# mpt0816/Cilqr

Hardware: AMD Instinct MI355X
Metric: CILQR solves/sec (50-step horizon, batch=65536 per GPU) (higher is better)
Workload: dtype f64

## Files before the change

cilqr_amd/csrc/backward_core.hpp:

```cpp
#pragma once
#include "dev_model.hpp"

namespace cilqr {

__host__ __device__ constexpr int a_kind(int r, int c) {
  return (r == c) ? 1
         : ((r == 0 || r == 1) && c >= 2) ? 2
         : (r == 2 && c >= 3) ? 2
         : (r == 3 && c == 4) ? 2
         : 0;
}
__host__ __device__ constexpr int b_kind(int r, int c) {
  return ((r == 2 && c == 1) || (r == 3 && c == 0) || (r == 4 && c == 0) || (r == 5 && c == 1)) ? 2 : 0;
}
__host__ __device__ constexpr int h_kind(int r, int c) {
  return (r < 3 && c < 3) ? 2 : (r == c) ? 2 : 0;
}

#define ACC_TERM(acc, t)            \
  do {                              \
    if ((acc).any) (acc).v += (t);  \
    else { (acc).v = (t); (acc).any = true; } \
  } while (0)

// ... 14 lines not shown
      const Acc a = acc_sum6_xty(t);
      out[r * xcols + c] = a.any ? a.v : 0.0;
    }
}
template <int C, int rows, bool IsA>
CILQR_DEV void x_m(const double* __restrict__ X, const double* __restrict__ M, double* out) {
#pragma unroll
  for (int r = 0; r < rows; ++r)
#pragma unroll
    for (int c = 0; c < C; ++c) {
      Acc a{0.0, false};
#pragma unroll
      for (int k = 0; k < 6; ++k) {
        const int kind = IsA ? a_kind(k, c) : b_kind(k, c);
        if (kind == 0) continue;
        const double x = X[r * 6 + k];
        const double t = (kind == 1) ? x : x * M[k * C + c];
        ACC_TERM(a, t);
      }
      out[r * C + c] = a.any ? a.v : 0.0;
    }
}

template <bool kStore>
CILQR_DEV void backward_problem(const DeviceState& s, int slot, double lambda, double2* stage) {
  const Params& p = s.p;
  const int Bc = s.Bcap, N = p.N;
  const double dt = p.dt;
  const int sp = scratch_index(s, slot);
  double Vx[6], Vxx[36];
  {
    const double2* t = s.term + sp;
    const double2 t0 = t[0], t1 = t[(size_t)Bc], t2 = t[(size_t)2 * Bc], t3 = t[(size_t)3 * Bc],
                  t4 = t[(size_t)4 * Bc], t5 = t[(size_t)5 * Bc], t6 = t[(size_t)6 * Bc],
                  t7 = t[(size_t)7 * Bc], t8 = t[(size_t)8 * Bc];
    Vx[0] = t0.x; Vx[1] = t0.y; Vx[2] = t1.x; Vx[3] = t1.y; Vx[4] = t2.x; Vx[5] = t2.y;
#pragma unroll
    for (int e = 0; e < 36; ++e) Vxx[e] = 0.0;
    Vxx[0] = t3.x; Vxx[1] = t3.y; Vxx[2] = t4.x;
    Vxx[6] = t4.y; Vxx[7] = t5.x; Vxx[8] = t5.y;
    Vxx[12] = t6.x; Vxx[13] = t6.y; Vxx[14] = t7.x;
    Vxx[21] = t7.y; Vxx[28] = t8.x; Vxx[35] = t8.y;
  }
  const int buf = s.cur[slot];
  double dV0 = 0.0, dV1 = 0.0, gsum = 0.0;
  double2 w[kLinPairs];
  double2 uu;
  constexpr int kRows = kLinPairs + 1;
  auto fetch_to_lds = [&](int step) {
    using gptr = const __attribute__((address_space(1))) void*;
    using lptr = __attribute__((address_space(3))) void*;
    const double2* q = s.lin + (size_t)step * kLinPairs * Bc + sp;
    double2* dst = stage + (size_t)(step & 1) * kRows * 64;
#pragma unroll
    for (int r = 0; r < kLinPairs; ++r)
      __builtin_amdgcn_global_load_lds((gptr)(q + (size_t)r * Bc), (lptr)(dst + r * 64), 16, 0, 0);
    __builtin_amdgcn_global_load_lds((gptr)(s.U + ((size_t)buf * N + step) * Bc + slot), (lptr)(dst + kLinPairs * 64), 16, 0, 0);
  };
  fetch_to_lds(N - 1);
  for (int i = N - 1; i >= 0; --i) {
    {
      asm volatile("s_waitcnt vmcnt(0)" ::: "memory");
      const double2* src = stage + (size_t)(i & 1) * kRows * 64 + (threadIdx.x & 63);
#pragma unroll
      for (int r = 0; r < kLinPairs; ++r) w[r] = src[r * 64];
      uu = src[kLinPairs * 64];
      if (i > 0) fetch_to_lds(i - 1);
    }
    double A[36], B[12];
    A[2] = w[0].x; A[3] = w[0].y; A[4] = w[1].x; A[5] = w[1].y;
    A[8] = w[2].x; A[9] = w[2].y; A[10] = w[3].x; A[11] = w[3].y;
    A[15] = w[4].x; A[16] = w[4].y; A[17] = w[5].x;
    A[22] = dt;
    B[5] = w[5].y; B[6] = 0.5 * dt * dt; B[8] = dt; B[11] = dt;
    const double lx[6] = {w[6].x, w[6].y, w[7].x, w[7].y, w[8].x, w[8].y};
    const double lu[2] = {w[9].x, w[9].y};
    double H[36];
    H[0] = w[10].x; H[1] = w[10].y; H[2] = w[11].x;
    H[6] = w[11].y; H[7] = w[12].x; H[8] = w[12].y;
    H[12] = w[13].x; H[13] = w[13].y; H[14] = w[14].x;
    H[21] = w[14].y; H[28] = w[15].x; H[35] = w[15].y;
    const double luu0 = w[16].x, luu1 = w[16].y;

    double BtV[12], Qux[12], BtVB[4], BtVx[2];
    mt_x<2, 6, false>(B, Vxx, BtV);
    x_m<6, 2, true>(BtV, A, Qux);
    x_m<2, 2, false>(BtV, B, BtVB);
    mt_x<2, 1, false>(B, Vx, BtVx);
    const double Quu[4] = {luu0 + BtVB[0], BtVB[1], BtVB[2], luu1 + BtVB[3]};
    const double Qu[2] = {lu[0] + BtVx[0], lu[1] + BtVx[1]};
    const double m00 = Quu[0] + lambda, m01 = Quu[1], m10 = Quu[2], m11 = Quu[3] + lambda;
    const double invdet = 1.0 / (m00 * m11 - m10 * m01);
    const double n00 = -(m11 * invdet), n01 = -(-m01 * invdet), n10 = -(-m10 * invdet),
                 n11 = -(m00 * invdet);
    double Kc[12], kc[2];
#pragma unroll
    for (int c = 0; c < 6; ++c) {
      Kc[c] = n00 * Qux[c] + n01 * Qux[6 + c];
      Kc[6 + c] = n10 * Qux[c] + n11 * Qux[6 + c];
    }
    kc[0] = n00 * Qu[0] + n01 * Qu[1];
    kc[1] = n10 * Qu[0] + n11 * Qu[1];
    if (kStore) {
      double2* g = s.gains + (size_t)i * kGainPairs * Bc + sp;
#pragma unroll
      for (int r = 0; r < 6; ++r) g[(size_t)r * Bc] = make_double2(Kc[2 * r], Kc[2 * r + 1]);
      g[(size_t)6 * Bc] = make_double2(kc[0], kc[1]);
    }
    {
      const double v0 = fabs(kc[0]) / (fabs(uu.x) + 1), v1 = fabs(kc[1]) / (fabs(uu.y) + 1);
      gsum += (v0 > v1 ? v0 : v1);
    }
    double AtVx[6], AtV[36], AtVA[36];
    mt_x<6, 1, true>(A, Vx, AtVx);
    mt_x<6, 6, true>(A, Vxx, AtV);
    x_m<6, 6, true>(AtV, A, AtVA);
    double KtQ[12];
#pragma unroll
    for (int r = 0; r < 6; ++r) {
      KtQ[r * 2 + 0] = Kc[r] * Quu[0] + Kc[6 + r] * Quu[2];
      KtQ[r * 2 + 1] = Kc[r] * Quu[1] + Kc[6 + r] * Quu[3];
    }
    double nVx[6];
#pragma unroll
    for (int r = 0; r < 6; ++r) {
      const double t1 = KtQ[r * 2] * kc[0] + KtQ[r * 2 + 1] * kc[1];
      const double t2 = Kc[r] * Qu[0] + Kc[6 + r] * Qu[1];
      const double t3 = Qux[r] * kc[0] + Qux[6 + r] * kc[1];
      nVx[r] = (((lx[r] + AtVx[r]) + t1) + t2) + t3;
    }
#pragma unroll
    for (int r = 0; r < 6; ++r)
#pragma unroll
      for (int c = 0; c < 6; ++c) {
        const double m1 = KtQ[r * 2] * Kc[c] + KtQ[r * 2 + 1] * Kc[6 + c];
        const double m2 = Kc[r] * Qux[c] + Kc[6 + r] * Qux[6 + c];
        const double m3 = Qux[r] * Kc[c] + Qux[6 + r] * Kc[6 + c];
        const double qxx = (h_kind(r, c) == 2) ? (H[r * 6 + c] + AtVA[r * 6 + c]) : AtVA[r * 6 + c];
        Vxx[r * 6 + c] = ((qxx + m1) + m2) + m3;
      }
#pragma unroll
    for (int r = 0; r < 6; ++r) Vx[r] = nVx[r];
#pragma unroll
    for (int c = 0; c < 6; ++c)
#pragma unroll
// ... 515 lines not shown
```

cilqr_amd/csrc/kernels_backward.hip:

```cpp
#include <hip/hip_ext.h>

#include "backward_core.hpp"

namespace cilqr {

__global__ __launch_bounds__(64) void k_backward_team(DeviceState s, const int* __restrict__ list, int n,
                                                      const double* __restrict__ lambda_override) {
  using namespace team;
  __shared__ double lds[(64 / kLanes) * kStride];
  const int lane = threadIdx.x;
  const int n_act = active_count(s, n);
  const int jraw = blockIdx.x * (64 / kLanes) + lane / kLanes;
  if ((int)(blockIdx.x * (64 / kLanes)) >= n_act) return;
  const bool live = jraw < n_act;
  const int j = live ? jraw : n_act - 1;
  const int slot = list ? list[j] : j;
  const double lambda = lambda_override ? lambda_override[slot] : s.lambda[slot];
  backward_team_problem(s, slot, lambda, live, lane & (kLanes - 1), lds + (lane / kLanes) * kStride, BlockSync{});
}

__global__ __launch_bounds__(64, 1) void k_backward(DeviceState s, const int* __restrict__ list, int n,
                                                     const double* __restrict__ lambda_override) {
  __shared__ double2 stage[2 * (kLinPairs + 1) * 64];
  const int j = blockIdx.x * blockDim.x + threadIdx.x;
  if (j >= active_count(s, n)) return;
  const int slot = list ? list[j] : j;
  const double lambda = lambda_override ? lambda_override[slot] : s.lambda[slot];
  backward_problem<true>(s, slot, lambda, stage);
}

bool launch_backward_wave(const DeviceState& s, const int* list, int n, const double* lambda_override, hipStream_t st,
                          hipEvent_t ev_start, hipEvent_t ev_stop);

void launch_backward(const DeviceState& s, const int* list, int n, const double* lambda_override,
                     int team_threshold, int wave_threshold, hipStream_t st, hipEvent_t ev_start, hipEvent_t ev_stop) {
  if (n == 0) return;
  if (n <= wave_threshold && launch_backward_wave(s, list, n, lambda_override, st, ev_start, ev_stop))
    return;
  if (n <= team_threshold)
    hipExtLaunchKernelGGL(k_backward_team, dim3((n + 7) / 8), dim3(64), 0, st, ev_start, ev_stop, 0, s, list, n, lambda_override);
  else
    hipExtLaunchKernelGGL(k_backward, dim3((n + 63) / 64), dim3(64), 0, st, ev_start, ev_stop, 0, s, list, n, lambda_override);
}

}
```

cilqr_amd/csrc/kernels_tail.hip:

```cpp
#include <algorithm>
#include <cstdlib>
#include <mutex>

#include "backward_core.hpp"
#include "quad_core.hpp"
#include "search_core.hpp"

namespace cilqr {

#ifndef CILQR_TAIL_THREADS
#define CILQR_TAIL_THREADS 256
#endif
constexpr int kTailThreads = CILQR_TAIL_THREADS;
constexpr int kTailChunk = 5;

struct TailLayout {
  size_t X, U, goals, cor, ccnt, lin, term, gains, Xs, Us, parts, spec_tot, dbl, ints, stride;
};
constexpr size_t kNotInLds = ~(size_t)0;
struct TailArgs {
  char* ws;
  TailLayout L;
  TailLayout S;
  int lds_base;
// ... 59 lines not shown
  t.parts = reinterpret_cast<double2*>(at(a.L.parts, a.S.parts));
  t.spec_tot = reinterpret_cast<double*>(at(a.L.spec_tot, a.S.spec_tot));
  double* d = reinterpret_cast<double*>(at(a.L.dbl, a.S.dbl));
  t.dV = d;
  t.gnorm = d + 2;
  t.trial = d + 3;
  t.lambda = d + 8;
  t.dlambda = d + 9;
  t.cost_old = d + 10;
  t.dcost = d + 11;
  int* q = reinterpret_cast<int*>(at(a.L.ints, a.S.ints));
  t.cur = q;
  t.pid = q + 1;
  t.done_now = q + 2;
  t.upd = q + 3;
  t.acc_idx = q + 4;
  t.emit = q + 5;
  t.part = nullptr;
  t.n_dev = nullptr;
  t.posn = nullptr;
  return t;
}

template <bool InLds>
__device__ __attribute__((noinline)) void tail_backward(int off_T, int off_view) {
  extern __shared__ double lds[];
  const DeviceState& t = *reinterpret_cast<const DeviceState*>(reinterpret_cast<const char*>(lds) + off_view);
  backward_wave_problem<WaveSync, true, InLds>(t, 0, t.lambda[0], (int)threadIdx.x, lds + off_T, WaveSync{});
}

#ifndef CILQR_TAIL_AHEAD
#define CILQR_TAIL_AHEAD 4
#endif
template <bool SrcLds, bool OutLds>
__device__ __attribute__((noinline)) void tail_forward(int off_view) {
  extern __shared__ double lds[];
  const DeviceState& t = *reinterpret_cast<const DeviceState*>(reinterpret_cast<const char*>(lds) + off_view);
  const int tid = (int)threadIdx.x;
  forward_core<OutSpecSolo<OutLds>, SrcLds ? 1 : CILQR_TAIL_AHEAD, true, SrcLds>(t, 0, kAlpha[tid], OutSpecSolo<OutLds>(t, tid));
}
template <int D, bool EX, bool InLds>
__device__ __attribute__((noinline)) void tail_quadratize(int off_view, int i) {
  extern __shared__ double lds[];
  const DeviceState& t = *reinterpret_cast<const DeviceState*>(reinterpret_cast<const char*>(lds) + off_view);
  knot_quadratize<D, EX, InLds>(t, lds, t.cur[0], i, 0);
}
constexpr int kQuadParts = 4;
template <bool EX>
__device__ __attribute__((noinline)) void tail_quad_items(int off_view, int off_scr, int cap, int i, int part) {
  extern __shared__ double lds[];
  const DeviceState& t = *reinterpret_cast<const DeviceState*>(reinterpret_cast<const char*>(lds) + off_view);
  knot_plane_items<EX, true>(t, lds, t.cur[0], i, part, kQuadParts, reinterpret_cast<double*>(reinterpret_cast<char*>(lds) + off_scr), cap,
                             quad_split_stride(cap));
}
__device__ __attribute__((noinline)) void tail_quad_commit(int off_view, int off_scr, int cap, int i) {
  extern __shared__ double lds[];
  const DeviceState& t = *reinterpret_cast<const DeviceState*>(reinterpret_cast<const char*>(lds) + off_view);
  knot_commit_items<true>(t, t.cur[0], i, reinterpret_cast<const double*>(reinterpret_cast<const char*>(lds) + off_scr), cap,
                          quad_split_stride(cap));
}
template <bool EX>
__device__ __attribute__((noinline)) void tail_quad_first_part(int off_view, int i) {
  extern __shared__ double lds[];
  const DeviceState& t = *reinterpret_cast<const DeviceState*>(reinterpret_cast<const char*>(lds) + off_view);
  knot_quadratize<5, EX, true, true>(t, lds, t.cur[0], i, 0);
}
template <int D, bool EX, bool InLds>
__device__ __attribute__((noinline)) void tail_knot_cost(int off_view, int r, int i) {
  extern __shared__ double lds[];
  const DeviceState& t = *reinterpret_cast<const DeviceState*>(reinterpret_cast<const char*>(lds) + off_view);
  const int K = t.p.K, N = t.p.N;
  const double2* xb = t.Xs + ((size_t)r * K + i) * 3;
  assume_lds<InLds>(xb);
  const double2 p0 = xb[0], p1 = xb[1], p2 = xb[2];
  const double x[6] = {p0.x, p0.y, p1.x, p1.y, p2.x, p2.y};
  double u[2] = {0.0, 0.0};
  if (i < N) {
    const double2* ub = t.Us + (size_t)r * N + i;
    assume_lds<InLds>(ub);
    const double2 q = *ub;
    u[0] = q.x; u[1] = q.y;
  }
  knot_cost<D, EX, InLds>(t, lds, i, 0, x, u, t.parts + ((size_t)r * K + i) * kPartPairs, 1);
}

#ifdef CILQR_TAIL_PROFILE
#define TP_DECL long long tp_[8] = {0, 0, 0, 0, 0, 0, 0, 0}; long long tp_t = __builtin_readcyclecounter(); int tp_it = 0;
#define TP(k) do { const long long n_ = __builtin_readcyclecounter(); tp_[k] += n_ - tp_t; tp_t = n_; } while (0)
#else
#define TP_DECL
#define TP(k)
#endif
#ifdef CILQR_TAIL_OCC
#define CILQR_TAIL_ATTR __attribute__((amdgpu_waves_per_eu(CILQR_TAIL_OCC, CILQR_TAIL_OCC)))
#else
#define CILQR_TAIL_ATTR
#endif
template <int D, bool EX>
__global__ __launch_bounds__(kTailThreads) CILQR_TAIL_ATTR void k_tail(DeviceState g, TailArgs a, int n_max) {
  extern __shared__ double lds[];
  const int n = active_count(g, n_max);
  const int blk = (gridDim.x & 63u) == 0 ? xcd_local_position((int)blockIdx.x) : (int)blockIdx.x;
  if (blk >= n) return;
  const int tid = threadIdx.x;
  (void)stage_lanes(g, lds);
  double* T = lds + ((g.nl + g.nr) * kLaneFields + 1) / 2 * 2;
  double* tot = T + wave::lds_doubles(g.p.N);
  int* flag = reinterpret_cast<int*>(tot + kNumAlpha * 5);
  DeviceState* tv = reinterpret_cast<DeviceState*>(flag + 16);
  if (tid == 0) *tv = tail_view(g, a, blk, reinterpret_cast<char*>(lds) + a.lds_base);
  __syncthreads();
  const DeviceState& t = *tv;
  const int off_view = (int)(reinterpret_cast<const char*>(tv) - reinterpret_cast<const char*>(lds));
  const int K = g.p.K, N = g.p.N;
  const size_t Bc = (size_t)g.Bcap;

  {
    const int src = g.act[blk];
    const int buf = g.cur[src];
    for (int i = tid; i < K; i += kTailThreads) {
      const double2* x = g.X + ((size_t)buf * K + i) * 3 * Bc + src;
      t.X[i * 3 + 0] = x[0];
// ... 12 lines not shown
      if (r < g.ccnt[(size_t)i * Bc + src] * 3) t.cor[i * rows_t + r] = g.cor[((size_t)i * rows + r) * Bc + src];
    }
    if (tid == 0) {
      t.cur[0] = 0;
      t.pid[0] = g.pid[src];
      t.lambda[0] = g.lambda[src];
      t.dlambda[0] = g.dlambda[src];
      t.cost_old[0] = g.cost_old[src];
      t.dcost[0] = g.dcost[src];
      t.upd[0] = 1;
      t.acc_idx[0] = -1;
      t.emit[0] = 0;
      t.done_now[0] = 0;
    }
  }
  __syncthreads();
  const int pb = t.pid[0];
  TP_DECL
  for (;;) {
    TP(7);
    if (t.upd[0]) {
      if (D == 5 && a.quad_scr >= 0) {
        const int off_scr = a.lds_base + a.quad_scr, cap = quad_split_planes(g.cmax);
        for (int w = tid; w < K * kQuadParts; w += kTailThreads) tail_quad_items<EX>(off_view, off_scr, cap, w / kQuadParts, w % kQuadParts);
        __syncthreads();
        const int wv = tid >> 6;
        for (int i = (wv >> 1) * 64 + (tid & 63); i < K; i += kTailThreads / 2) {
          if (wv & 1) tail_quad_first_part<EX>(off_view, i);
          else tail_quad_commit(off_view, off_scr, cap, i);
        }
      } else if (a.quad_in_lds) { for (int i = tid; i < K; i += kTailThreads) tail_quadratize<D, EX, true>(off_view, i); }
      else { for (int i = tid; i < K; i += kTailThreads) tail_quadratize<D, EX, false>(off_view, i); }
    }
    __syncthreads();
    TP(0);
    if (tid < 64) {
      if (a.bwd_in_lds) tail_backward<true>((int)(T - lds), off_view);
      else tail_backward<false>((int)(T - lds), off_view);
    }
    __syncthreads();
    TP(1);
    if (tid == 0) {
      const bool leave = leaves_before_search(t, 0, true);
      t.acc_idx[0] = leave ? -2 : -1;
      flag[0] = leave ? 1 : 0;
      flag[1] = -1;
    }
    __syncthreads();
    if (!flag[0]) {
      if (tid < kNumAlpha) {
        if (a.fwd_in_lds) tail_forward<true, true>(off_view);
        else if (a.fwd_src_in_lds) tail_forward<true, false>(off_view);
        else tail_forward<false, false>(off_view);
      }
      __syncthreads();
      TP(2);
      int acc = -1;
      for (int r0 = 0; r0 < kNumAlpha && acc < 0; r0 += kTailChunk) {
        const int nr = min(kTailChunk, kNumAlpha - r0);
        for (int e = tid; e < nr * K; e += kTailThreads) {
          const int rr = e / K, i = e - rr * K, r = r0 + rr;
          if (a.cost_in_lds) tail_knot_cost<D, EX, true>(off_view, r, i);
          else tail_knot_cost<D, EX, false>(off_view, r, i);
        }
        __syncthreads();
        TP(3);
        if (tid < nr) {
          const int r = r0 + tid;
          double jj = 0.0, dx = 0.0, du = 0.0, cc = 0.0, lc = 0.0;
          const double2* pp = t.parts + (size_t)r * K * kPartPairs;
#pragma unroll 8
          for (int i = 0; i < K; ++i) {
            const double2* o = pp + (size_t)i * kPartPairs;
            const double2 aa = o[0], c2 = o[2];
            jj += aa.x;
            dx += aa.y;
            cc += c2.x;
            lc += c2.y;
          }
#pragma unroll 8
          for (int i = 0; i < N; ++i) {
            const double2 bb = pp[(size_t)i * kPartPairs + 1];
            jj += bb.x;
            du += bb.y;
          }
          const double dyn = dx + du;
// ... 58 lines not shown
#endif
    if (a.iter_trajs && t.emit[0]) {
      const int idx = g.n_iter_trajs[pb] - 1;
      if (idx < a.it_cap)
        for (int i = tid; i < K; i += kTailThreads)
          write_traj_point(t, t.cur[0], i, 0, a.iter_trajs + (((size_t)pb * a.it_cap + idx) * K + i) * 10);
    }
    if (done) {
      for (int i = tid; i < K; i += kTailThreads)
        write_traj_point(t, t.cur[0], i, 0, a.traj + ((size_t)pb * K + i) * 10);
      if (tid == 0) atomicMax(a.max_iter, g.iter[pb]);
      break;
    }
  }
}

static size_t tail_fixed_lds(const DeviceState& g) {
  const size_t lane_d = (size_t)((g.nl + g.nr) * kLaneFields + 1) / 2 * 2;
  return ((lane_d + wave::lds_doubles(g.p.N) + kNumAlpha * 5) * sizeof(double) + 16 * sizeof(int) + sizeof(DeviceState) + 31) / 16 * 16;
}
bool tail_supported(const DeviceState& g) { return tail_fixed_lds(g) <= 62 * 1024; }

void launch_tail(const DeviceState& g, void* workspace, int n_max, double* traj, double* iter_trajs,
                 int max_iter_trajs, int* max_iter_dev, hipStream_t st) {
  if (n_max <= 0) return;
  TailArgs a;
  a.ws = static_cast<char*>(workspace);
  a.L = tail_layout(g);
  a.traj = traj;
  a.iter_trajs = iter_trajs;
  a.it_cap = max_iter_trajs;
  a.max_iter = max_iter_dev;
  const size_t fixed = tail_fixed_lds(g);
  struct DeviceLds { std::once_flag once; size_t bytes = 0; };
  static DeviceLds lds_of[64];
  int dev = 0;
  (void)hipGetDevice(&dev);
  DeviceLds& dl = lds_of[dev & 63];
  std::call_once(dl.once, [&] {
    int max_lds = 0;
    if (hipDeviceGetAttribute(&max_lds, hipDeviceAttributeMaxSharedMemoryPerBlock, dev) != hipSuccess || max_lds <= 0) max_lds = 64 * 1024;
    const void* fns[] = {reinterpret_cast<const void*>(&k_tail<5, false>), reinterpret_cast<const void*>(&k_tail<5, true>),
                         reinterpret_cast<const void*>(&k_tail<0, false>), reinterpret_cast<const void*>(&k_tail<0, true>)};
    bool ok = true;
    for (const void* f : fns) ok = ok && hipFuncSetAttribute(f, hipFuncAttributeMaxDynamicSharedMemorySize, max_lds) == hipSuccess;
    if (!ok) {
      (void)hipGetLastError();
      max_lds = std::min(max_lds, 64 * 1024);
    }
    dl.bytes = (size_t)max_lds;
  });
  const size_t budget = dl.bytes > fixed + 2048 ? dl.bytes - 2048 - fixed : 0;
  const size_t K = g.p.K, N = g.p.N;
  struct Item { size_t TailLayout::*field; size_t bytes; };
  const Item items[] = {
      {&TailLayout::dbl, 16 * sizeof(double)}, {&TailLayout::ints, 8 * sizeof(int)}, {&TailLayout::spec_tot, (size_t)kNumAlpha * 5 * sizeof(double)},
      {&TailLayout::term, kTermPairs * sizeof(double2)}, {&TailLayout::gains, N * kGainPairs * sizeof(double2)},
      {&TailLayout::X, 2 * K * 3 * sizeof(double2)}, {&TailLayout::U, 2 * N * sizeof(double2)},
      {&TailLayout::lin, N * kLinPairs * sizeof(double2)}, {&TailLayout::parts, (size_t)kNumAlpha * K * kPartPairs * sizeof(double2)},
      {&TailLayout::Xs, (size_t)kNumAlpha * K * 3 * sizeof(double2)}, {&TailLayout::Us, (size_t)kNumAlpha * N * sizeof(double2)},
      {&TailLayout::goals, K * 3 * sizeof(double2)}, {&TailLayout::ccnt, K * sizeof(int)}, {&TailLayout::cor, K * tail_cmax(g.cmax) * 3 * sizeof(double)}};
  size_t used = 0;
  a.S = a.L;
  for (const Item& it : items) {
    const size_t b = (it.bytes + 15) / 16 * 16;
    if (used + b <= budget) { a.S.*(it.field) = used; used += b; }
// ... 2 lines not shown
  a.lds_base = (int)fixed;
  auto in_lds = [&](size_t TailLayout::*f) { return a.S.*f != kNotInLds; };
  a.bwd_in_lds = in_lds(&TailLayout::lin) && in_lds(&TailLayout::term) && in_lds(&TailLayout::gains) && in_lds(&TailLayout::U) &&
                 in_lds(&TailLayout::dbl);
  a.fwd_src_in_lds = in_lds(&TailLayout::X) && in_lds(&TailLayout::U) && in_lds(&TailLayout::gains) && in_lds(&TailLayout::goals);
  a.fwd_in_lds = a.fwd_src_in_lds && in_lds(&TailLayout::Xs) && in_lds(&TailLayout::Us);
  a.quad_in_lds = in_lds(&TailLayout::X) && in_lds(&TailLayout::U) && in_lds(&TailLayout::goals) && in_lds(&TailLayout::cor) &&
                  in_lds(&TailLayout::ccnt) && in_lds(&TailLayout::lin) && in_lds(&TailLayout::term);
  a.cost_in_lds = in_lds(&TailLayout::Xs) && in_lds(&TailLayout::Us) && in_lds(&TailLayout::parts) && in_lds(&TailLayout::goals) &&
                  in_lds(&TailLayout::cor) && in_lds(&TailLayout::ccnt);
  {
    auto al = [](size_t b) { return (b + 15) / 16 * 16; };
    const size_t b_parts = al((size_t)kNumAlpha * K * kPartPairs * sizeof(double2)), b_xs = al((size_t)kNumAlpha * K * 3 * sizeof(double2)),
                 b_us = al((size_t)kNumAlpha * N * sizeof(double2));
    const bool one_piece = in_lds(&TailLayout::parts) && in_lds(&TailLayout::Xs) && in_lds(&TailLayout::Us) &&
                           a.S.Xs == a.S.parts + b_parts && a.S.Us == a.S.Xs + b_xs;
    const size_t need = K * (size_t)quad_split_doubles(g.cmax) * sizeof(double);
    const char* env = std::getenv("CILQR_TAIL_QUAD_SPLIT");
    const bool off = env && env[0] == '0';
    a.quad_scr = (!off && g.p.num_of_disc == 5 && a.quad_in_lds && one_piece && need <= b_parts + b_xs + b_us && kTailThreads == 256)
                     ? (int)a.S.parts : -1;
  }
  const size_t lds = fixed + used;
  if (g.p.num_of_disc == 5) {
    if (g.exact_ties) hipLaunchKernelGGL((k_tail<5, true>), dim3(n_max >= 64 ? (n_max + 63) / 64 * 64 : n_max), dim3(kTailThreads), lds, st, g, a, n_max);
    else hipLaunchKernelGGL((k_tail<5, false>), dim3(n_max >= 64 ? (n_max + 63) / 64 * 64 : n_max), dim3(kTailThreads), lds, st, g, a, n_max);
  } else {
    if (g.exact_ties) hipLaunchKernelGGL((k_tail<0, true>), dim3(n_max >= 64 ? (n_max + 63) / 64 * 64 : n_max), dim3(kTailThreads), lds, st, g, a, n_max);
    else hipLaunchKernelGGL((k_tail<0, false>), dim3(n_max >= 64 ? (n_max + 63) / 64 * 64 : n_max), dim3(kTailThreads), lds, st, g, a, n_max);
  }
}

}
```

cilqr_amd/csrc/search_core.hpp:

```cpp
#pragma once
#include "cost_reduce.hpp"

namespace cilqr {

static __device__ const double kAlpha[kNumAlpha] = {1.0000, 0.5012, 0.2512, 0.1259, 0.0631, 0.0316,
                                             0.0158, 0.0079, 0.0040, 0.0020, 0.0010};


struct OutSlot {
  const DeviceState& s;
  int nb, slot;
  CILQR_DEV void x(int i, const double* v) const { store_x(s, nb, i, slot, v); }
  CILQR_DEV void u(int i, const double* v) const { store_u(s, nb, i, slot, v); }
};
struct OutSpec {
  const DeviceState& s;
  int r, j;
  CILQR_DEV void x(int i, const double* v) const {
    const size_t cap = (size_t)s.spec_cap;
    double2* b = s.Xs + ((size_t)r * s.p.K + i) * 3 * cap + j;
    b[0] = make_double2(v[0], v[1]);
    b[cap] = make_double2(v[2], v[3]);
    b[2 * cap] = make_double2(v[4], v[5]);
  }
// ... 3 lines not shown
};

template <bool InLds>
struct OutSpecSolo {
  double2* xs;
  double2* us;
  CILQR_DEV OutSpecSolo(const DeviceState& s, int r) : xs(s.Xs + (size_t)r * s.p.K * 3), us(s.Us + (size_t)r * s.p.N) {
    assume_lds<InLds>(xs);
    assume_lds<InLds>(us);
  }
  CILQR_DEV void x(int i, const double* v) const {
    double2* b = xs + (size_t)i * 3;
    b[0] = make_double2(v[0], v[1]);
    b[1] = make_double2(v[2], v[3]);
    b[2] = make_double2(v[4], v[5]);
  }
  CILQR_DEV void u(int i, const double* v) const { us[i] = make_double2(v[0], v[1]); }
};

#ifndef CILQR_ROLL_AHEAD
#define CILQR_ROLL_AHEAD 4
#endif
constexpr int kFwdAhead = CILQR_ROLL_AHEAD;
struct FwdStep {
  double2 x0, x1, x2, u, kk[kGainPairs];
};
struct FwdSrc {
  const double2* X;
  const double2* U;
  const double2* gains;
  size_t Bc;
};
CILQR_DEV FwdSrc fwd_source(const DeviceState& s, int buf, int slot, int sp, size_t Bc) {
  return FwdSrc{s.X + (size_t)buf * s.p.K * 3 * Bc + slot, s.U + (size_t)buf * s.p.N * Bc + slot, s.gains + sp, Bc};
}
CILQR_DEV void load_fwd_step(const FwdSrc& q, int i, FwdStep& f) {
  const double2* b = q.X + (size_t)i * 3 * q.Bc;
  f.x0 = b[0]; f.x1 = b[q.Bc]; f.x2 = b[2 * q.Bc];
  f.u = q.U[(size_t)i * q.Bc];
  const double2* g = q.gains + (size_t)i * kGainPairs * q.Bc;
#pragma unroll
  for (int r = 0; r < kGainPairs; ++r) f.kk[r] = g[(size_t)r * q.Bc];
}

template <class Out, int kAhead = kFwdAhead, bool Solo = false, bool InLds = false>
CILQR_DEV void forward_core(const DeviceState& s, int slot, double alpha, const Out& out) {
  const DynP p = dyn_params(s.p);
  const size_t Bc = Solo ? (size_t)1 : (size_t)s.Bcap;
  const int N = s.p.N;
  const int buf = s.cur[slot];
  const int sp = Solo ? 0 : scratch_index(s, slot);
  double x[6];
  {
    const double2* gp = s.goals + slot;
    const double2 g0 = gp[0], g1 = gp[Bc], g2 = gp[2 * Bc];
    x[0] = g0.x; x[1] = g0.y; x[2] = g1.x; x[3] = g1.y; x[4] = g2.x; x[5] = g2.y;
  }
  const FwdSrc src = fwd_source(s, buf, slot, sp, Bc);
  assume_lds<InLds>(src.X);
  assume_lds<InLds>(src.U);
  assume_lds<InLds>(src.gains);
  out.x(0, x);
  FwdStep pf[kAhead];
#pragma unroll
  for (int d = 0; d < kAhead; ++d)
    if (d < N) load_fwd_step(src, d, pf[d]);
  for (int i0 = 0; i0 < N; i0 += kAhead) {
#pragma unroll
// ... 159 lines not shown
```

cilqr_amd/csrc/solver.hip:

```cpp
#include <hip/hip_runtime.h>

#include <dlfcn.h>
#include <pthread.h>

#include <chrono>
#include <cmath>
#include <condition_variable>
#include <cstdio>
#include <mutex>
#include <thread>
#include <cstdlib>
#include <cstring>
#include <memory>
#include <new>
#include <vector>

#include "build_id.h"
#include "solver_priv.hpp"

using namespace cilqr;

void cilqr_comm_release(cilqr_solver* h);

thread_local char g_last_hip_error[256] = "";
// ... 732 lines not shown

static int solve_one(cilqr_solver* h, cilqr_job& j, const cilqr_problem_batch* in, cilqr_solution_batch* out) {
  if (in) j.in = *in; else std::memset(&j.in, 0, sizeof(j.in));
  j.out = *out;
  j.upload = 0;
  j.zero_inline = true;
  int rc = (in == nullptr) ? CILQR_ERR_NULL : job_begin(h, j);
  if (rc == CILQR_OK) rc = job_iterate(h, j, 1);
  if (rc == CILQR_OK && j.handed) rc = job_iterate(h, j, 2);
  if (rc == CILQR_OK) rc = job_finish(h, j);
  else {
    (void)hipStreamSynchronize(j.st1);
    if (j.st2 != j.st1) (void)hipStreamSynchronize(j.st2);
  }
  release_fin(h, j);
  return rc;
}

static int solve_sync(cilqr_solver* h, const cilqr_problem_batch* in, cilqr_solution_batch* out) {
  cilqr_job& j = h->jobs[0];
  j.set = 0;
  j.spec_threshold = h->spec_threshold;
  j.tail_threshold = h->tail_threshold;
  j.st1 = h->stream;
  j.st2 = h->stream;
  j.relaxed_wait = false;
  const int rc = solve_groups(h, j, in, out);
  std::lock_guard<std::mutex> lk(h->mu);
  h->prof = j.prof;
  return rc;
}

static int solve_groups(cilqr_solver* h, cilqr_job& j, const cilqr_problem_batch* in, cilqr_solution_batch* out) {
  if (in == nullptr || in->n_lane_groups <= 1) return solve_one(h, j, in, out);
  if (in->lane_group_start == nullptr || in->lane_group_left == nullptr || in->lane_group_right == nullptr ||
      in->left_lane == nullptr || in->right_lane == nullptr)
    return CILQR_ERR_CONSTRAINTS;
  if (in->lane_group_start[0] != 0 || in->lane_group_start[in->n_lane_groups] != in->batch) return CILQR_ERR_ARG;
  const size_t K = (size_t)in->n_knots, M1 = (size_t)h->cfg.max_iter + 1;
  size_t lrow = 0, rrow = 0;
  cilqr_profile acc;
  std::memset(&acc, 0, sizeof(acc));
  for (int g = 0; g < in->n_lane_groups; ++g) {
    const int b0 = in->lane_group_start[g], b1 = in->lane_group_start[g + 1];
    if (b1 < b0 || in->lane_group_left[g] <= 0 || in->lane_group_right[g] <= 0) return CILQR_ERR_ARG;
    if (b1 > b0) {
// ... 230 lines not shown
      DeviceState f = h->fin;
      adopt_job_fields(&f, j.gmain);
      launch_compact(a, f, n_hint, st);
      hipLaunchKernelGGL(k_seed_counters, dim3(1), dim3(64), 0, st, f.counters, a.n_next, kCntActive + it % 3);
      HIP_TRY(hipGetLastError());
      if (j.tm.end()) return CILQR_ERR_DEVICE;
      HIP_TRY(hipEventRecord(js.handoff.get(), st));
      d = f;
      o = twin_of(f, h->fin_twin);
      j.span = n_hint;
      j.handed = true;
      j.owns_fin = true;
      return CILQR_OK;
    }
    d.n_dev = d.counters + kCntActive + it % 3;
    d.n_next = d.counters + kCntActive + (it + 1) % 3;
    d.n_clear = d.counters + kCntActive + (it + 2) % 3;
    d.h_count_dev = js.h_count_dev + it;
    o.n_dev = d.n_dev; o.n_next = d.n_next; o.n_clear = d.n_clear; o.h_count_dev = d.h_count_dev;
    if (n_hint <= tail_threshold) {
      void* ws = (stage == 1 && !j.handed) ? h->tail_ws1.get() : h->tail_ws.get();
      if (j.tm.begin(4)) return CILQR_ERR_DEVICE;
      HIP_TRY(hipMemsetAsync(js.tail_iter_dev, 0, sizeof(int), st));
      launch_tail(d, ws, n_hint, j.o_traj, j.o_it, j.out.max_iter_trajs, js.tail_iter_dev, st);
      HIP_TRY(hipMemcpyAsync(h_count + M + 32, js.tail_iter_dev, sizeof(int), hipMemcpyDeviceToHost, st));
      if (j.tm.end()) return CILQR_ERR_DEVICE;
      j.tail_used = true;
      j.tail_n = n_hint;
      break;
    }
    if (j.tm.begin(0)) return CILQR_ERR_DEVICE;
    launch_quadratize(d, d.act, n_hint, 0, st);
    hipEvent_t eb0, eb1;
    if (j.tm.end() || j.tm.pair(1, &eb0, &eb1)) return CILQR_ERR_DEVICE;
    cilqr_phase_mark_begin(1);
    launch_backward(d, d.act, n_hint, nullptr, h->team_threshold, h->wave_threshold, st, eb0, eb1);
    cilqr_phase_mark_end();
    if (j.tm.begin(2)) return CILQR_ERR_DEVICE;
    j.bwd_iter.push_back(it);
    launch_linesearch(d, n_hint, j.spec_threshold, h->seq_rounds, h->round_group, st);
    launch_update(d, n_hint, st);
    launch_export_done(d, n_hint, j.o_traj, st);
    if (j.o_it) launch_export_iter_traj(d, d.act, n_hint, j.o_it, j.out.max_iter_trajs, st);
    if (j.tm.end()) return CILQR_ERR_DEVICE;
    HIP_TRY(hipEventRecord(js.iter_ev[it].get(), st));
    if (h->compaction && (int64_t)100 * n_hint <= (int64_t)h->compact_percent * j.span) {
      if (j.tm.begin(3)) return CILQR_ERR_DEVICE;
// ... 306 lines not shown
}

extern "C" {

int cilqr_submit(cilqr_handle h, const cilqr_problem_batch* in, cilqr_solution_batch* out) {
  if (h == nullptr || in == nullptr || out == nullptr) return CILQR_ERR_NULL;
  std::lock_guard<std::mutex> lk(h->mu);
  if (h->job_count >= kJobRing) return CILQR_ERR_STATE;
  if (!h->workers_started) {
    h->worker1 = std::thread(worker1_main, h);
    h->worker2 = std::thread(worker2_main, h);
    h->worker_io = std::thread(worker_io_main, h);
    h->workers_started = true;
  }
  const int slot = (h->job_head + h->job_count) % kJobRing;
  cilqr_job& j = h->jobs[slot];
  j.in = *in;
  j.out = *out;
  j.set = 0;
  j.in_buf = -1;
  j.past_load = false;
  j.spec_threshold = h->alone_on_device ? h->spec_threshold : h->spec_threshold_submit;
  j.tail_threshold = h->alone_on_device ? h->tail_threshold : h->tail_threshold_submit;
  j.st1 = h->stream;
  j.st2 = h->stream2.get();
  j.relaxed_wait = true;
  const bool plain = in->n_lane_groups <= 1 && in->batch > 0 && in->batch <= h->capacity;
  j.upload = (plain && in->memory == CILQR_MEM_HOST && check_problem(h, in) == CILQR_OK &&
              input_payload_bytes(h, in) > kSmallTransfer) ? 1 : 0;
  j.zero_by_io = plain && out->cost_hist != nullptr && host_out_is_big(h, in->batch, out);
  j.zero_inline = !j.zero_by_io;
  j.io_busy = j.upload == 1 || j.zero_by_io;
  j.io_taken = false;
  j.upload_rc = CILQR_OK;
  j.rc = CILQR_OK;
  j.err_text[0] = 0;
  j.phase = 1;
  h->job_count += 1;
  h->cv.notify_all();
  return CILQR_OK;
}

int cilqr_wait(cilqr_handle h) {
  if (h == nullptr) return CILQR_ERR_NULL;
  std::unique_lock<std::mutex> lk(h->mu);
  if (h->job_count == 0) return CILQR_ERR_STATE;
// ... 241 lines not shown
```

cilqr_amd/csrc/solver_priv.hpp:

```cpp
#pragma once
#include <atomic>

#include <hip/hip_runtime.h>

#include <condition_variable>
#include <cstdio>
#include <mutex>
#include <thread>
#include <vector>

#include "../../include/cilqr.h"
#include "hip_owned.hpp"
#include "state.hpp"

extern thread_local char g_last_hip_error[256];

#define HIP_TRY(expr)                                                              \
  do {                                                                             \
    hipError_t e_ = (expr);                                                        \
    if (e_ != hipSuccess) {                                                        \
      std::snprintf(g_last_hip_error, sizeof(g_last_hip_error), "%s -> %s", #expr, \
                    hipGetErrorString(e_));                                        \
      return CILQR_ERR_DEVICE;                                                     \
    }                                                                              \
// ... 46 lines not shown
  bool wants(int k) const;
  int reserve();
  int begin(int k);
  int pair(int k, hipEvent_t* a, hipEvent_t* b);
  int end();
  void resolve(cilqr_profile* p);
};

struct cilqr_in_buffer {
  cilqr::dev_mem p;
  cilqr::hip_event ready;
  cilqr::hip_event loaded;
  int state = 0;
};

constexpr int kJobRing = 3;

struct cilqr_job {
  cilqr_problem_batch in;
  cilqr_solution_batch out;
  int set = 0;
  int spec_threshold = 0;
  int tail_threshold = 0;
  int phase = 0;
  int rc = CILQR_OK;
  char err_text[256] = "";
  hipStream_t st1 = nullptr, st2 = nullptr;
  cilqr::DeviceState gmain;
  cilqr::DeviceState d, o;
  int B = 0, it = 0, n_hint = 0, span = 0;
  bool handed = false;
  bool owns_fin = false;
  bool tail_used = false;
  int tail_n = 0;
  std::vector<int> bwd_iter;
  cilqr_timer tm;
  cilqr_profile prof;
  double *o_traj = nullptr, *o_hist = nullptr, *o_it = nullptr;
  int *o_nc = nullptr, *o_st = nullptr, *o_ni = nullptr, *o_nit = nullptr;
  signed char* o_at = nullptr;
  size_t n_traj = 0, n_hist = 0, n_itr = 0, n_at = 0;
  size_t n_head = 0;
  bool small_out = false;
  bool relaxed_wait = false;
  int upload = 0;
  int upload_rc = CILQR_OK;
// ... 84 lines not shown
```

cilqr_amd/csrc/state.hpp:

```cpp
#pragma once

#include <hip/hip_runtime.h>
#include <stdint.h>

namespace cilqr {

constexpr int kNX = 6;
constexpr int kNU = 2;
constexpr int kLinPairs = 17;
constexpr int kTermPairs = 9;
constexpr int kGainPairs = 7;
constexpr int kPartPairs = 3;
constexpr int kNumAlpha = 11;
constexpr int kMaxDiscs = 16;
constexpr int kLaneFields = 11;
constexpr int kGridCellBytes = 16;
#ifndef CILQR_GRID_CELLS_LOG2
#define CILQR_GRID_CELLS_LOG2 16
#endif
constexpr int kGridMaxCells = 1 << CILQR_GRID_CELLS_LOG2;
constexpr int kGridFullScan = 255;

constexpr int kRowA = 0, kRowLx = 6, kRowLu = 9, kRowH = 10, kRowLuu = 16;
constexpr int kDenseDoublesPerStep = 110;
// ... 110 lines not shown
void launch_init_guess(const DeviceState& s, int B, hipStream_t st);
void launch_init_guess_tracker(const DeviceState& s, const TrackerParams& tp, int B, hipStream_t st);
void launch_set_trajectory(const DeviceState& s, int B, const double* X, const double* U, hipStream_t st);
void launch_cost_only(const DeviceState& s, const int* list, int n, int cand, hipStream_t st);
void launch_cost_knots(const DeviceState& s, const int* list, const int* n_ptr, int n_max, int n_grid,
                       int cand, int skip_done, hipStream_t st);
void launch_spec_cost(const DeviceState& s, const int* list, const int* n_ptr, int off, int n_max, int n_grid, int r0,
                      int sparse, hipStream_t st);
int spec_open_capacity(const DeviceState& s);
void launch_round_cost(const DeviceState& s, int r0, int group, int n_max, int n_grid, hipStream_t st);
void launch_init_cost_commit(const DeviceState& s, int n, hipStream_t st);
void launch_quadratize(const DeviceState& s, const int* list, int n, int only_upd, hipStream_t st);
void launch_backward(const DeviceState& s, const int* list, int n, const double* lambda_override,
                     int team_threshold, int wave_threshold, hipStream_t st, hipEvent_t ev_start = nullptr,
                     hipEvent_t ev_stop = nullptr);
void launch_forward(const DeviceState& s, const int* list, int n, double alpha, int skip_done,
                    hipStream_t st);
void launch_linesearch(const DeviceState& s, int n_act, int spec_threshold, int seq_rounds, int round_group,
                       hipStream_t st);
void launch_init_counters(const DeviceState& s, int first_n, hipStream_t st);
size_t tail_workspace_bytes(const DeviceState& s);
bool tail_supported(const DeviceState& s);
void launch_tail(const DeviceState& s, void* workspace, int n_max, double* traj, double* iter_trajs,
                 int max_iter_trajs, int* max_iter_dev, hipStream_t st);
void launch_update(const DeviceState& s, int n_act, hipStream_t st);
void launch_export_done(const DeviceState& s, int n_act, double* traj, hipStream_t st);
void launch_compact(const DeviceState& src, const DeviceState& dst, int n_max, hipStream_t st);
void launch_export_iter_traj(const DeviceState& s, const int* list, int n, double* iter_trajs,
                             int max_iter_trajs, hipStream_t st);
void launch_export_hist(const DeviceState& s, int B, double* cost_hist, int* n_cost, int* status,
                        int* n_iter, int* n_iter_trajs, signed char* alpha_trace, hipStream_t st);
void launch_export_hist_rows(const DeviceState& s, int B, long long* off, double* rows, hipStream_t st);
constexpr int kCorMaxPts = 320;
struct CorridorParams {
  double max_diff_x, max_diff_y, radius, max_axis_x, max_axis_y;
  int per_edge;
};
void launch_build_corridors(int n, const CorridorParams& cp, const double* knots, const double* points,
                            const int* count, int pmax, double* corridor, int* ccount, int cmax, int* n_failed,
                            double* polygons, hipStream_t st);
struct DpParams;
void launch_dp_place(const DpParams& P, int first, int n_scenes, const double* dyn_poly, const int* dyn_poly_counts,
                     const double* dyn_traj, const int* dyn_traj_counts, double* placed, int* placed_n, hipStream_t st);
void launch_dp_plan(const DpParams& P, int first, int n_scenes, const double* start3, const double* static_points,
                    const int* static_counts, const int* dyn_poly_counts, const int* dyn_traj_counts, const double* placed,
                    const int* placed_n, double* coarse9, double* coarse6, double* knots3, double* station, int* found,
                    int* n_not_found, hipStream_t st);
// ... 11 lines not shown
```

Baseline: 2.133 million.

## Shrink backward LDS staging, defer cost loads, tune tail occupancy and forward lookahead

The backward kernel now stages the control row in one shared slot instead of double-buffering it, which shrinks LDS use. It also loads the lx and H cost rows only after the gain computation, aiming to lower peak register pressure. The tail kernel gets a Beside template variant with different waves-per-EU bounds, chosen when the solver is not alone on the device. The default forward lookahead changes from 4 to 3 (CILQR_ROLL_AHEAD_LANE). The risks are a race on the single control slot and extra LDS read latency in the middle of the loop.

```diff
diff --git a/cilqr_amd/csrc/backward_core.hpp b/cilqr_amd/csrc/backward_core.hpp
--- a/cilqr_amd/csrc/backward_core.hpp
+++ b/cilqr_amd/csrc/backward_core.hpp
@@ -60,6 +60,7 @@
     }
 }
 
+constexpr int kBwdStageRows = 2 * kLinPairs + 1;
 template <bool kStore>
 CILQR_DEV void backward_problem(const DeviceState& s, int slot, double lambda, double2* stage) {
   const Params& p = s.p;
@@ -84,25 +85,28 @@
   double dV0 = 0.0, dV1 = 0.0, gsum = 0.0;
   double2 w[kLinPairs];
   double2 uu;
-  constexpr int kRows = kLinPairs + 1;
+  double2* const urow = stage + (size_t)2 * kLinPairs * 64;
   auto fetch_to_lds = [&](int step) {
     using gptr = const __attribute__((address_space(1))) void*;
     using lptr = __attribute__((address_space(3))) void*;
     const double2* q = s.lin + (size_t)step * kLinPairs * Bc + sp;
-    double2* dst = stage + (size_t)(step & 1) * kRows * 64;
+    double2* dst = stage + (size_t)(step & 1) * kLinPairs * 64;
 #pragma unroll
     for (int r = 0; r < kLinPairs; ++r)
       __builtin_amdgcn_global_load_lds((gptr)(q + (size_t)r * Bc), (lptr)(dst + r * 64), 16, 0, 0);
-    __builtin_amdgcn_global_load_lds((gptr)(s.U + ((size_t)buf * N + step) * Bc + slot), (lptr)(dst + kLinPairs * 64), 16, 0, 0);
+    __builtin_amdgcn_global_load_lds((gptr)(s.U + ((size_t)buf * N + step) * Bc + slot), (lptr)urow, 16, 0, 0);
   };
   fetch_to_lds(N - 1);
   for (int i = N - 1; i >= 0; --i) {
-    {
-      asm volatile("s_waitcnt vmcnt(0)" ::: "memory");
-      const double2* src = stage + (size_t)(i & 1) * kRows * 64 + (threadIdx.x & 63);
-#pragma unroll
-      for (int r = 0; r < kLinPairs; ++r) w[r] = src[r * 64];
-      uu = src[kLinPairs * 64];
+    asm volatile("s_waitcnt vmcnt(0)" ::: "memory");
+    const double2* src = stage + (size_t)(i & 1) * kLinPairs * 64 + (threadIdx.x & 63);
+    {
+#pragma unroll
+      for (int r = 0; r < 6; ++r) w[r] = src[r * 64];
+      w[kRowLu] = src[kRowLu * 64];
+      w[kRowLuu] = src[kRowLuu * 64];
+      uu = urow[threadIdx.x & 63];
+      asm volatile("s_waitcnt lgkmcnt(0)" ::: "memory");
       if (i > 0) fetch_to_lds(i - 1);
     }
     double A[36], B[12];
@@ -111,14 +115,8 @@
     A[15] = w[4].x; A[16] = w[4].y; A[17] = w[5].x;
     A[22] = dt;
     B[5] = w[5].y; B[6] = 0.5 * dt * dt; B[8] = dt; B[11] = dt;
-    const double lx[6] = {w[6].x, w[6].y, w[7].x, w[7].y, w[8].x, w[8].y};
-    const double lu[2] = {w[9].x, w[9].y};
-    double H[36];
-    H[0] = w[10].x; H[1] = w[10].y; H[2] = w[11].x;
-    H[6] = w[11].y; H[7] = w[12].x; H[8] = w[12].y;
-    H[12] = w[13].x; H[13] = w[13].y; H[14] = w[14].x;
-    H[21] = w[14].y; H[28] = w[15].x; H[35] = w[15].y;
-    const double luu0 = w[16].x, luu1 = w[16].y;
+    const double lu[2] = {w[kRowLu].x, w[kRowLu].y};
+    const double luu0 = w[kRowLuu].x, luu1 = w[kRowLuu].y;
 
     double BtV[12], Qux[12], BtVB[4], BtVx[2];
     mt_x<2, 6, false>(B, Vxx, BtV);
@@ -159,6 +157,16 @@
       KtQ[r * 2 + 0] = Kc[r] * Quu[0] + Kc[6 + r] * Quu[2];
       KtQ[r * 2 + 1] = Kc[r] * Quu[1] + Kc[6 + r] * Quu[3];
     }
+#pragma unroll
+    for (int r = 6; r < 9; ++r) w[r] = src[r * 64];
+#pragma unroll
+    for (int r = 10; r < 16; ++r) w[r] = src[r * 64];
+    const double lx[6] = {w[6].x, w[6].y, w[7].x, w[7].y, w[8].x, w[8].y};
+    double H[36];
+    H[0] = w[10].x; H[1] = w[10].y; H[2] = w[11].x;
+    H[6] = w[11].y; H[7] = w[12].x; H[8] = w[12].y;
+    H[12] = w[13].x; H[13] = w[13].y; H[14] = w[14].x;
+    H[21] = w[14].y; H[28] = w[15].x; H[35] = w[15].y;
     double nVx[6];
 #pragma unroll
     for (int r = 0; r < 6; ++r) {
diff --git a/cilqr_amd/csrc/kernels_backward.hip b/cilqr_amd/csrc/kernels_backward.hip
--- a/cilqr_amd/csrc/kernels_backward.hip
+++ b/cilqr_amd/csrc/kernels_backward.hip
@@ -21,7 +21,7 @@
 
 __global__ __launch_bounds__(64, 1) void k_backward(DeviceState s, const int* __restrict__ list, int n,
                                                      const double* __restrict__ lambda_override) {
-  __shared__ double2 stage[2 * (kLinPairs + 1) * 64];
+  __shared__ double2 stage[kBwdStageRows * 64];
   const int j = blockIdx.x * blockDim.x + threadIdx.x;
   if (j >= active_count(s, n)) return;
   const int slot = list ? list[j] : j;
diff --git a/cilqr_amd/csrc/kernels_tail.hip b/cilqr_amd/csrc/kernels_tail.hip
--- a/cilqr_amd/csrc/kernels_tail.hip
+++ b/cilqr_amd/csrc/kernels_tail.hip
@@ -105,7 +105,7 @@
   return t;
 }
 
-template <bool InLds>
+template <bool InLds, bool Beside>
 __device__ __attribute__((noinline)) void tail_backward(int off_T, int off_view) {
   extern __shared__ double lds[];
   const DeviceState& t = *reinterpret_cast<const DeviceState*>(reinterpret_cast<const char*>(lds) + off_view);
@@ -115,40 +115,41 @@
 #ifndef CILQR_TAIL_AHEAD
 #define CILQR_TAIL_AHEAD 4
 #endif
-template <bool SrcLds, bool OutLds>
+template <bool SrcLds, bool OutLds, bool Beside>
 __device__ __attribute__((noinline)) void tail_forward(int off_view) {
   extern __shared__ double lds[];
   const DeviceState& t = *reinterpret_cast<const DeviceState*>(reinterpret_cast<const char*>(lds) + off_view);
   const int tid = (int)threadIdx.x;
   forward_core<OutSpecSolo<OutLds>, SrcLds ? 1 : CILQR_TAIL_AHEAD, true, SrcLds>(t, 0, kAlpha[tid], OutSpecSolo<OutLds>(t, tid));
 }
-template <int D, bool EX, bool InLds>
+template <int D, bool EX, bool InLds, bool Beside>
 __device__ __attribute__((noinline)) void tail_quadratize(int off_view, int i) {
   extern __shared__ double lds[];
   const DeviceState& t = *reinterpret_cast<const DeviceState*>(reinterpret_cast<const char*>(lds) + off_view);
   knot_quadratize<D, EX, InLds>(t, lds, t.cur[0], i, 0);
 }
 constexpr int kQuadParts = 4;
-template <bool EX>
+template <bool EX, bool Beside>
 __device__ __attribute__((noinline)) void tail_quad_items(int off_view, int off_scr, int cap, int i, int part) {
   extern __shared__ double lds[];
   const DeviceState& t = *reinterpret_cast<const DeviceState*>(reinterpret_cast<const char*>(lds) + off_view);
   knot_plane_items<EX, true>(t, lds, t.cur[0], i, part, kQuadParts, reinterpret_cast<double*>(reinterpret_cast<char*>(lds) + off_scr), cap,
                              quad_split_stride(cap));
 }
+template <bool Beside>
 __device__ __attribute__((noinline)) void tail_quad_commit(int off_view, int off_scr, int cap, int i) {
   extern __shared__ double lds[];
   const DeviceState& t = *reinterpret_cast<const DeviceState*>(reinterpret_cast<const char*>(lds) + off_view);
   knot_commit_items<true>(t, t.cur[0], i, reinterpret_cast<const double*>(reinterpret_cast<const char*>(lds) + off_scr), cap,
                           quad_split_stride(cap));
 }
-template <bool EX>
+template <bool EX, bool Beside>
 __device__ __attribute__((noinline)) void tail_quad_first_part(int off_view, int i) {
   extern __shared__ double lds[];
   const DeviceState& t = *reinterpret_cast<const DeviceState*>(reinterpret_cast<const char*>(lds) + off_view);
   knot_quadratize<5, EX, true, true>(t, lds, t.cur[0], i, 0);
 }
-template <int D, bool EX, bool InLds>
+template <int D, bool EX, bool InLds, bool Beside>
 __device__ __attribute__((noinline)) void tail_knot_cost(int off_view, int r, int i) {
   extern __shared__ double lds[];
   const DeviceState& t = *reinterpret_cast<const DeviceState*>(reinterpret_cast<const char*>(lds) + off_view);
@@ -175,12 +176,13 @@
 #define TP(k)
 #endif
 #ifdef CILQR_TAIL_OCC
-#define CILQR_TAIL_ATTR __attribute__((amdgpu_waves_per_eu(CILQR_TAIL_OCC, CILQR_TAIL_OCC)))
+#define CILQR_TAIL_WAVES(beside) CILQR_TAIL_OCC, CILQR_TAIL_OCC
 #else
-#define CILQR_TAIL_ATTR
+#define CILQR_TAIL_WAVES(beside) (beside) ? 2 : 1, (beside) ? 2 : 8
 #endif
-template <int D, bool EX>
-__global__ __launch_bounds__(kTailThreads) CILQR_TAIL_ATTR void k_tail(DeviceState g, TailArgs a, int n_max) {
+template <int D, bool EX, bool Beside>
+__global__ __launch_bounds__(kTailThreads) __attribute__((amdgpu_waves_per_eu(CILQR_TAIL_WAVES(Beside))))
+void k_tail(DeviceState g, TailArgs a, int n_max) {
   extern __shared__ double lds[];
   const int n = active_count(g, n_max);
   const int blk = (gridDim.x & 63u) == 0 ? xcd_local_position((int)blockIdx.x) : (int)blockIdx.x;
@@ -239,21 +241,21 @@
     if (t.upd[0]) {
       if (D == 5 && a.quad_scr >= 0) {
         const int off_scr = a.lds_base + a.quad_scr, cap = quad_split_planes(g.cmax);
-        for (int w = tid; w < K * kQuadParts; w += kTailThreads) tail_quad_items<EX>(off_view, off_scr, cap, w / kQuadParts, w % kQuadParts);
+        for (int w = tid; w < K * kQuadParts; w += kTailThreads) tail_quad_items<EX, Beside>(off_view, off_scr, cap, w / kQuadParts, w % kQuadParts);
         __syncthreads();
         const int wv = tid >> 6;
         for (int i = (wv >> 1) * 64 + (tid & 63); i < K; i += kTailThreads / 2) {
-          if (wv & 1) tail_quad_first_part<EX>(off_view, i);
-          else tail_quad_commit(off_view, off_scr, cap, i);
+          if (wv & 1) tail_quad_first_part<EX, Beside>(off_view, i);
+          else tail_quad_commit<Beside>(off_view, off_scr, cap, i);
         }
-      } else if (a.quad_in_lds) { for (int i = tid; i < K; i += kTailThreads) tail_quadratize<D, EX, true>(off_view, i); }
-      else { for (int i = tid; i < K; i += kTailThreads) tail_quadratize<D, EX, false>(off_view, i); }
+      } else if (a.quad_in_lds) { for (int i = tid; i < K; i += kTailThreads) tail_quadratize<D, EX, true, Beside>(off_view, i); }
+      else { for (int i = tid; i < K; i += kTailThreads) tail_quadratize<D, EX, false, Beside>(off_view, i); }
     }
     __syncthreads();
     TP(0);
     if (tid < 64) {
-      if (a.bwd_in_lds) tail_backward<true>((int)(T - lds), off_view);
-      else tail_backward<false>((int)(T - lds), off_view);
+      if (a.bwd_in_lds) tail_backward<true, Beside>((int)(T - lds), off_view);
+      else tail_backward<false, Beside>((int)(T - lds), off_view);
     }
     __syncthreads();
     TP(1);
@@ -266,9 +268,9 @@
     __syncthreads();
     if (!flag[0]) {
       if (tid < kNumAlpha) {
-        if (a.fwd_in_lds) tail_forward<true, true>(off_view);
-        else if (a.fwd_src_in_lds) tail_forward<true, false>(off_view);
-        else tail_forward<false, false>(off_view);
+        if (a.fwd_in_lds) tail_forward<true, true, Beside>(off_view);
+        else if (a.fwd_src_in_lds) tail_forward<true, false, Beside>(off_view);
+        else tail_forward<false, false, Beside>(off_view);
       }
       __syncthreads();
       TP(2);
@@ -277,8 +279,8 @@
         const int nr = min(kTailChunk, kNumAlpha - r0);
         for (int e = tid; e < nr * K; e += kTailThreads) {
           const int rr = e / K, i = e - rr * K, r = r0 + rr;
-          if (a.cost_in_lds) tail_knot_cost<D, EX, true>(off_view, r, i);
-          else tail_knot_cost<D, EX, false>(off_view, r, i);
+          if (a.cost_in_lds) tail_knot_cost<D, EX, true, Beside>(off_view, r, i);
+          else tail_knot_cost<D, EX, false, Beside>(off_view, r, i);
         }
         __syncthreads();
         TP(3);
@@ -383,7 +385,7 @@
 bool tail_supported(const DeviceState& g) { return tail_fixed_lds(g) <= 62 * 1024; }
 
 void launch_tail(const DeviceState& g, void* workspace, int n_max, double* traj, double* iter_trajs,
-                 int max_iter_trajs, int* max_iter_dev, hipStream_t st) {
+                 int max_iter_trajs, int* max_iter_dev, bool beside, hipStream_t st) {
   if (n_max <= 0) return;
   TailArgs a;
   a.ws = static_cast<char*>(workspace);
@@ -401,8 +403,10 @@
   std::call_once(dl.once, [&] {
     int max_lds = 0;
     if (hipDeviceGetAttribute(&max_lds, hipDeviceAttributeMaxSharedMemoryPerBlock, dev) != hipSuccess || max_lds <= 0) max_lds = 64 * 1024;
-    const void* fns[] = {reinterpret_cast<const void*>(&k_tail<5, false>), reinterpret_cast<const void*>(&k_tail<5, true>),
-                         reinterpret_cast<const void*>(&k_tail<0, false>), reinterpret_cast<const void*>(&k_tail<0, true>)};
+    const void* fns[] = {reinterpret_cast<const void*>(&k_tail<5, false, false>), reinterpret_cast<const void*>(&k_tail<5, true, false>),
+                         reinterpret_cast<const void*>(&k_tail<0, false, false>), reinterpret_cast<const void*>(&k_tail<0, true, false>),
+                         reinterpret_cast<const void*>(&k_tail<5, false, true>), reinterpret_cast<const void*>(&k_tail<5, true, true>),
+                         reinterpret_cast<const void*>(&k_tail<0, false, true>), reinterpret_cast<const void*>(&k_tail<0, true, true>)};
     bool ok = true;
     for (const void* f : fns) ok = ok && hipFuncSetAttribute(f, hipFuncAttributeMaxDynamicSharedMemorySize, max_lds) == hipSuccess;
     if (!ok) {
@@ -451,13 +455,15 @@
                      ? (int)a.S.parts : -1;
   }
   const size_t lds = fixed + used;
+  const dim3 grid(n_max >= 64 ? (n_max + 63) / 64 * 64 : n_max);
+  auto launch = [&](auto kernel) { hipLaunchKernelGGL(kernel, grid, dim3(kTailThreads), lds, st, g, a, n_max); };
   if (g.p.num_of_disc == 5) {
-    if (g.exact_ties) hipLaunchKernelGGL((k_tail<5, true>), dim3(n_max >= 64 ? (n_max + 63) / 64 * 64 : n_max), dim3(kTailThreads), lds, st, g, a, n_max);
-    else hipLaunchKernelGGL((k_tail<5, false>), dim3(n_max >= 64 ? (n_max + 63) / 64 * 64 : n_max), dim3(kTailThreads), lds, st, g, a, n_max);
+    if (g.exact_ties) beside ? launch(k_tail<5, true, true>) : launch(k_tail<5, true, false>);
+    else beside ? launch(k_tail<5, false, true>) : launch(k_tail<5, false, false>);
   } else {
-    if (g.exact_ties) hipLaunchKernelGGL((k_tail<0, true>), dim3(n_max >= 64 ? (n_max + 63) / 64 * 64 : n_max), dim3(kTailThreads), lds, st, g, a, n_max);
-    else hipLaunchKernelGGL((k_tail<0, false>), dim3(n_max >= 64 ? (n_max + 63) / 64 * 64 : n_max), dim3(kTailThreads), lds, st, g, a, n_max);
-  }
-}
-
-}
+    if (g.exact_ties) beside ? launch(k_tail<0, true, true>) : launch(k_tail<0, true, false>);
+    else beside ? launch(k_tail<0, false, true>) : launch(k_tail<0, false, false>);
+  }
+}
+
+}
diff --git a/cilqr_amd/csrc/search_core.hpp b/cilqr_amd/csrc/search_core.hpp
--- a/cilqr_amd/csrc/search_core.hpp
+++ b/cilqr_amd/csrc/search_core.hpp
@@ -49,6 +49,10 @@
 #define CILQR_ROLL_AHEAD 4
 #endif
 constexpr int kFwdAhead = CILQR_ROLL_AHEAD;
+#ifndef CILQR_ROLL_AHEAD_LANE
+#define CILQR_ROLL_AHEAD_LANE 3
+#endif
+constexpr int kFwdAheadLane = CILQR_ROLL_AHEAD_LANE;
 struct FwdStep {
   double2 x0, x1, x2, u, kk[kGainPairs];
 };
@@ -70,7 +74,7 @@
   for (int r = 0; r < kGainPairs; ++r) f.kk[r] = g[(size_t)r * q.Bc];
 }
 
-template <class Out, int kAhead = kFwdAhead, bool Solo = false, bool InLds = false>
+template <class Out, int kAhead = kFwdAheadLane, bool Solo = false, bool InLds = false>
 CILQR_DEV void forward_core(const DeviceState& s, int slot, double alpha, const Out& out) {
   const DynP p = dyn_params(s.p);
   const size_t Bc = Solo ? (size_t)1 : (size_t)s.Bcap;
diff --git a/cilqr_amd/csrc/solver.hip b/cilqr_amd/csrc/solver.hip
--- a/cilqr_amd/csrc/solver.hip
+++ b/cilqr_amd/csrc/solver.hip
@@ -778,6 +778,7 @@
   j.set = 0;
   j.spec_threshold = h->spec_threshold;
   j.tail_threshold = h->tail_threshold;
+  j.tail_beside = false;
   j.st1 = h->stream;
   j.st2 = h->stream;
   j.relaxed_wait = false;
@@ -1054,7 +1055,7 @@
       void* ws = (stage == 1 && !j.handed) ? h->tail_ws1.get() : h->tail_ws.get();
       if (j.tm.begin(4)) return CILQR_ERR_DEVICE;
       HIP_TRY(hipMemsetAsync(js.tail_iter_dev, 0, sizeof(int), st));
-      launch_tail(d, ws, n_hint, j.o_traj, j.o_it, j.out.max_iter_trajs, js.tail_iter_dev, st);
+      launch_tail(d, ws, n_hint, j.o_traj, j.o_it, j.out.max_iter_trajs, js.tail_iter_dev, j.tail_beside, st);
       HIP_TRY(hipMemcpyAsync(h_count + M + 32, js.tail_iter_dev, sizeof(int), hipMemcpyDeviceToHost, st));
       if (j.tm.end()) return CILQR_ERR_DEVICE;
       j.tail_used = true;
@@ -1407,6 +1408,7 @@
   j.past_load = false;
   j.spec_threshold = h->alone_on_device ? h->spec_threshold : h->spec_threshold_submit;
   j.tail_threshold = h->alone_on_device ? h->tail_threshold : h->tail_threshold_submit;
+  j.tail_beside = !h->alone_on_device;
   j.st1 = h->stream;
   j.st2 = h->stream2.get();
   j.relaxed_wait = true;
diff --git a/cilqr_amd/csrc/solver_priv.hpp b/cilqr_amd/csrc/solver_priv.hpp
--- a/cilqr_amd/csrc/solver_priv.hpp
+++ b/cilqr_amd/csrc/solver_priv.hpp
@@ -92,6 +92,7 @@
   int set = 0;
   int spec_threshold = 0;
   int tail_threshold = 0;
+  bool tail_beside = false;
   int phase = 0;
   int rc = CILQR_OK;
   char err_text[256] = "";
diff --git a/cilqr_amd/csrc/state.hpp b/cilqr_amd/csrc/state.hpp
--- a/cilqr_amd/csrc/state.hpp
+++ b/cilqr_amd/csrc/state.hpp
@@ -156,7 +156,7 @@
 size_t tail_workspace_bytes(const DeviceState& s);
 bool tail_supported(const DeviceState& s);
 void launch_tail(const DeviceState& s, void* workspace, int n_max, double* traj, double* iter_trajs,
-                 int max_iter_trajs, int* max_iter_dev, hipStream_t st);
+                 int max_iter_trajs, int* max_iter_dev, bool beside, hipStream_t st);
 void launch_update(const DeviceState& s, int n_act, hipStream_t st);
 void launch_export_done(const DeviceState& s, int n_act, double* traj, hipStream_t st);
 void launch_compact(const DeviceState& src, const DeviceState& dst, int n_max, hipStream_t st);
```

Measured after the change: 2.070 million. -2.9%, worse.
